# QData/LaMP

Measured on AMD Instinct MI355X. Metric: forward samples/sec, reuters d512 2+2L 4h, higher is better.
Workload: dtype f32

## Files before the change

include/lamp_hip.h:

```cpp
#ifndef LAMP_HIP_H
#define LAMP_HIP_H

#include <stddef.h>
#include <stdint.h>

#ifdef __cplusplus
extern "C" {
#endif
#if defined(__GNUC__)
#pragma GCC visibility push(default)
#endif

#define LAMP_HIP_ABI_VERSION 5

typedef void* lamp_stream_t;

enum lamp_status {
    LAMP_OK = 0,
    LAMP_E_DIMS = -1,
    LAMP_E_ALIGN = -2,
    LAMP_E_WORKSPACE = -3,
    LAMP_E_UNSUPPORTED = -4,
    LAMP_E_NULL = -5
};
// ... 314 lines not shown
    const float* slf_v;
} lamp_dec_gemm_pack;
typedef struct lamp_enc_gemm_pack {
    const float* w1;
    const float* w2;
} lamp_enc_gemm_pack;
typedef struct lamp_gemm_packs {
    const lamp_enc_gemm_pack* enc;
    const lamp_dec_gemm_pack* dec;
} lamp_gemm_packs;

int lamp_forward_packs(const lamp_model* m, const lamp_fwd_options* opts, const lamp_gemm_packs* packs, const int64_t* src_seq,
                       const int64_t* src_pos, int32_t B, int32_t T, float* logits, float* enc_output, const lamp_aux* aux,
                       void* workspace, size_t workspace_bytes, lamp_stream_t stream);

typedef struct lamp_onehot_frontend {
    const float* t1;
    const float* conv1_b;
    const float* conv2_w;
    const float* conv2_b;
    const float* conv2_pack;
    int32_t n_vocab;
    int32_t taps;
} lamp_onehot_frontend;

size_t lamp_onehot_forward_workspace_bytes(const lamp_model* m, const lamp_onehot_frontend* fe, int32_t micro_batch, int32_t T,
                                           int32_t want_attn);
int lamp_onehot_forward(const lamp_model* m, const lamp_onehot_frontend* fe, const int64_t* src_seq, const int64_t* src_pos,
                        int32_t B, int32_t T, float* logits, float* enc_output, const lamp_aux* aux, void* workspace,
                        size_t workspace_bytes, lamp_stream_t stream);
// ... 74 lines not shown
```

lamp_amd/Models.py:

```python
import ctypes as C

import collections

import torch
import torch.nn as nn

from . import _native as N
from .Decoders import GraphDecoder, MLPDecoder, RNNDecoder
from .Encoders import GraphEncoder, MLPEncoder, RNNEncoder
from .SubLayers import XavierLinear


def _chain_pack(fc, w1, w2, keep):
    ptrs = []
    for fmt in (0, 1):
        trio = [N.weight_pack(w, fmt) for w in (fc, w1, w2)]
        if any(t is None for t in trio):
            trio = [None] * 3
        keep.append(trio)
        ptrs += [N.ptr(t) for t in trio]
    return N.ChainPack(*ptrs)


class _MatmulPrecision:
# ... 166 lines not shown

    def _enc_chain_weights(self):
        out = []
        for l in self.encoder.layer_stack:
            if getattr(l.slf_attn, 'fc', None) is not None:
                out += [l.slf_attn.fc.weight, l.pos_ffn.w_1.weight, l.pos_ffn.w_2.weight]
        return out

    def _gemm_pack_weights(self):
        enc = [(l.pos_ffn.w_1.weight, l.pos_ffn.w_2.weight) for l in self.encoder.layer_stack]
        dec = []
        for l in self.decoder.layer_stack:
            slf = getattr(l, 'slf_attn', None)
            dec.append((l.enc_attn.w_qs.weight,) + (tuple(getattr(slf, n).weight for n in ('w_qs', 'w_ks', 'w_vs')) if slf is not None
                                                     else (None, None, None)))
        return enc, dec

    def _native_model(self):
        replica = getattr(self, '_is_replica', False)
        params = None if replica else self._param_list
        if params is None:
            params = self._weight_tensors()
            if not replica:
                self._param_list = params
        mask = self.decoder.label_mask_u8
        tiles = self.decoder.label_tiles
        bits = self.decoder.label_mask_bits
        bias = self.decoder.current_label_bias()
        if bias is not None:
            mask, tiles, bits = bias, None, None
        hoist = self.cache_layer0_query and not replica
        packs = self.use_chain_packs and not replica
        onehot = bool(getattr(self.encoder, 'onehot', False))
        live = self.enc_self_attn
        gpacks = bool(self.use_gemm_packs and not replica and not onehot and getattr(N.lib(), 'lamp_forward_packs', None))
        fold = self.fold_embedding and not replica and len(self.encoder.layer_stack) > 0 and not onehot and not live
        sparse = bool(self.use_sparse_label_attention and self.use_mask_bits and self.decoder.label_rows_sparse and bias is None)
        key = tuple(p.data_ptr() for p in params) + (N.ptr(mask), N.ptr(bits), N.ptr(tiles), self.use_label_tiles,
                                                      hoist, self.use_mask_bits, packs, fold, sparse, live, bias is not None, gpacks)
        if hoist:
            l0 = self.decoder.layer_stack[0].enc_attn
            key += (self.decoder.tgt_word_emb.weight._version, l0.w_qs.weight._version)
        if packs:
            key += tuple(w._version for w in self._chain_weights())
            if live:
                key += tuple(w._version for w in self._enc_chain_weights())
        if gpacks:
            key += tuple(w._version for group in self._gemm_pack_weights() for ws in group for w in ws if w is not None)
        if fold:
            key += tuple(w._version for w in self._fold_weights() if w is not None)
        if onehot:
            key += tuple((w.data_ptr(), w._version) for w in self._onehot_weights())
        cache = None if replica else self._native_cache
        if cache is not None and cache[0] == key:
# ... 36 lines not shown
                        continue
                    pack_arr[2 * i + j] = _chain_pack(att.fc.weight, ff.w_1.weight, ff.w_2.weight, pack_keep)
            m.chain_packs = pack_arr
            torch.cuda.current_stream().synchronize()
        enc_pack_arr = None
        if packs and live and len(enc.layer_stack) > 0:
            enc_pack_arr = (N.ChainPack * len(enc.layer_stack))()
            pack_keep = pack_keep if pack_keep is not None else []
            for i, l in enumerate(enc.layer_stack):
                if getattr(l.slf_attn, 'fc', None) is None:
                    continue
                enc_pack_arr[i] = _chain_pack(l.slf_attn.fc.weight, l.pos_ffn.w_1.weight, l.pos_ffn.w_2.weight, pack_keep)
            torch.cuda.current_stream().synchronize()
        gemm_keep = None
        if gpacks:
            enc_ws, dec_ws = self._gemm_pack_weights()
            tensors = []

            def pk(w):
                t = N.weight_pack(w, 0) if w is not None else None
                tensors.append(t)
                return N.ptr(t)
            enc_gp = (N.EncGemmPack * max(1, len(enc_ws)))(*[N.EncGemmPack(*[pk(w) for w in ws]) for ws in enc_ws])
            dec_gp = (N.DecGemmPack * max(1, len(dec_ws)))(*[N.DecGemmPack(*[pk(w) for w in ws]) for ws in dec_ws])
            gemm_keep = (N.GemmPacks(enc_gp, dec_gp), enc_gp, dec_gp, tensors)
            torch.cuda.current_stream().synchronize()
        fold_keep = None
        if fold:
            emb_w, pos_w, w1, b1 = self._fold_weights()
            w1 = w1.detach().reshape(w1.size(0), -1)
            e1 = N.linear(emb_w.detach(), w1, None if pos_w is not None else b1.detach())
            p1 = N.linear(pos_w.detach(), w1, b1.detach()) if pos_w is not None else None
            m.enc0_emb_w1, m.enc0_pos_w1 = e1.data_ptr(), N.ptr(p1)
            fold_keep = (e1, p1)
            torch.cuda.current_stream().synchronize()
        onehot_keep = None
        if onehot:
            e_w, w1, b1, w2, b2 = (w.detach() for w in self._onehot_weights())
            t1 = N.onehot_tap_table(e_w, w1)
            w2c, b1c, b2c = N.f32c(w2), N.f32c(b1), N.f32c(b2)
# ... 129 lines not shown
            def ws_bytes(mb):
                return lib.lamp_onehot_forward_workspace_bytes(C.byref(model), C.byref(fe), mb, T_in, int(want_attn))
        else:
            def ws_bytes(mb):
                return lib.lamp_forward_workspace_bytes(C.byref(model), mb, T, int(want_attn))
        per_sample = ws_bytes(1)
        fixed = 2 * per_sample - ws_bytes(2)
        whole = fixed + (per_sample - fixed) * B + 4096
        budget = max(per_sample + 4096, min(whole, self.workspace_limit_bytes))
        ws = N.workspace(budget, dev)
        if opts is not None and fe is not None:
            N.check(lib.lamp_onehot_forward_opts(C.byref(model), C.byref(fe), C.byref(opts), seq.data_ptr(), pos.data_ptr(), B,
                                                 T_in, logits.data_ptr(), enc_output.data_ptr(),
                                                 C.byref(aux) if aux is not None else None, ws.data_ptr(), ws.numel(),
                                                 N.stream()), 'lamp_onehot_forward_opts')
        elif gp is not None and fe is None:
            N.check(lib.lamp_forward_packs(C.byref(model), C.byref(opts) if opts is not None else None, C.byref(gp), seq.data_ptr(),
                                           pos.data_ptr(), B, T, logits.data_ptr(), enc_output.data_ptr(),
                                           C.byref(aux) if aux is not None else None, ws.data_ptr(), ws.numel(), N.stream()),
                    'lamp_forward_packs')
        elif opts is not None:
            N.check(lib.lamp_forward_opts(C.byref(model), C.byref(opts), seq.data_ptr(), pos.data_ptr(), B, T,
                                          logits.data_ptr(), enc_output.data_ptr(), C.byref(aux) if aux is not None else None,
                                          ws.data_ptr(), ws.numel(), N.stream()), 'lamp_forward_opts')
        elif fe is not None:
            N.check(lib.lamp_onehot_forward(C.byref(model), C.byref(fe), seq.data_ptr(), pos.data_ptr(), B, T_in,
                                            logits.data_ptr(), enc_output.data_ptr(), C.byref(aux) if aux is not None else None,
                                            ws.data_ptr(), ws.numel(), N.stream()), 'lamp_onehot_forward')
        else:
            N.check(lib.lamp_forward(C.byref(model), seq.data_ptr(), pos.data_ptr(), B, T, logits.data_ptr(),
# ... 14 lines not shown
        if was_training:
            self.eval()
        try:
            with torch.no_grad(), torch.cuda.device(src[0].device):
                logits = self.forward(src, adj, None, None)[0]
                idx, val = metrics.topk_labels(logits, k, values=True)
                return torch.sigmoid(val), idx.long()
        finally:
            if was_training:
                self.train(True)

    workspace_limit_bytes = 8 << 30
    cache_layer0_query = True
    use_chain_packs = True
    use_gemm_packs = True
    fold_embedding = True
    matmul_precision = _MatmulPrecision()
    use_packed_live_encoder = False
    use_label_tiles = True
    use_sparse_label_attention = True
    use_mask_bits = True
```

lamp_amd/_native.py:

```python
import ctypes as C
import os
import threading

import torch

_HERE = os.path.dirname(os.path.abspath(__file__))
LIB_PATH = os.environ.get('LAMP_HIP_LIBRARY') or os.path.join(_HERE, 'liblamp_hip.so')
TUNING_LIB_PATH = os.path.join(_HERE, 'liblamp_hip_tuning.so')

ABI_VERSION = 5
LAMP_MASK_NONE, LAMP_MASK_U8, LAMP_MASK_KEY_TOKENS_I64, LAMP_MASK_BITS_U32 = 0, 1, 2, 3
LAMP_MASK_BIAS_F32 = 4
LAMP_MASK_SPARSE_ROWS, LAMP_MASK_SELF_RAGGED = 1, 2
LAMP_FWD_PACKED_ENCODER, LAMP_FWD_DEC_SIGMOID = 1, 2
LAMP_FWD_MATMUL_BF16X3, LAMP_FWD_MATMUL_BF16X6 = 4, 8
LAMP_FWD_LABEL_BIAS = 16
LAMP_PREC_FP32, LAMP_PREC_BF16X3, LAMP_PREC_BF16X6 = 0, 1, 2
MATMUL_PRECISIONS = {'highest': (LAMP_PREC_FP32, 0), 'high': (LAMP_PREC_BF16X3, LAMP_FWD_MATMUL_BF16X3),
                     'bf16x6': (LAMP_PREC_BF16X6, LAMP_FWD_MATMUL_BF16X6)}
LAMP_ATTN_SOFTMAX, LAMP_ATTN_SIGMOID = 0, 1
ATTN_TYPES = {'softmax': LAMP_ATTN_SOFTMAX, 'sigmoid': LAMP_ATTN_SIGMOID}
K_EMBED, K_GEMM, K_ATTN, K_LAYERNORM, K_DIAG, K_COUNT = 0, 1, 2, 3, 4, 5
KERNEL_CLASS_NAMES = ('embed', 'gemm', 'attention', 'layernorm', 'diag_readout')

# ... 46 lines not shown
    _fields_ = [('n_src_vocab', C.c_int32), ('n_position', C.c_int32), ('n_labels', C.c_int32),
                ('d_model', C.c_int32), ('d_inner', C.c_int32), ('d_k', C.c_int32), ('d_v', C.c_int32),
                ('n_layers_enc', C.c_int32), ('n_layers_dec', C.c_int32), ('label_mask_flags', C.c_int32),
                ('src_word_emb', _vp), ('position_enc', _vp), ('tgt_word_emb', _vp), ('w_out', _vp),
                ('label_mask', _vp), ('label_mask_bits', _vp), ('label_tiles', _vp), ('enc_layers', C.POINTER(EncLayer)), ('dec_layers', C.POINTER(DecLayer)),
                ('dec0_query', _vp), ('chain_packs', C.POINTER(ChainPack)),
                ('enc0_emb_w1', _vp), ('enc0_pos_w1', _vp), ('label_mask_allowed', C.c_int64)]


class DecGemmPack(C.Structure):
    _fields_ = [('enc_q', _vp), ('slf_q', _vp), ('slf_k', _vp), ('slf_v', _vp)]


class EncGemmPack(C.Structure):
    _fields_ = [('w1', _vp), ('w2', _vp)]


class GemmPacks(C.Structure):
    _fields_ = [('enc', C.POINTER(EncGemmPack)), ('dec', C.POINTER(DecGemmPack))]


class GemmDesc(C.Structure):
    _fields_ = [('A', _vp), ('B', _vp), ('C', _vp), ('M', C.c_int32), ('N', C.c_int32), ('K', C.c_int32),
                ('batch0', C.c_int32), ('batch1', C.c_int32), ('accumulate', C.c_int32),
                ('a_row_stride', C.c_int64), ('a_col_stride', C.c_int64), ('a_batch0', C.c_int64), ('a_batch1', C.c_int64),
                ('b_row_stride', C.c_int64), ('b_col_stride', C.c_int64), ('b_batch0', C.c_int64), ('b_batch1', C.c_int64),
                ('ldc', C.c_int64), ('c_batch0', C.c_int64), ('c_batch1', C.c_int64),
                ('relu_mask', _vp), ('ld_mask', C.c_int64), ('alpha', C.c_float), ('reserved', C.c_int32)]


# ... 78 lines not shown
    'lamp_attn_bias_bwd': (C.c_int, [_vp, _i64, _i32, _i32, _f, _vp, _i64, _vp, _i64, _vp, _sz, _vp]),
    'lamp_label_bias_fold': (C.c_int, [_vp, _i64, _vp, _i32, _vp, _vp]),
    'lamp_dropout': (C.c_int, [_vp, _i64, _f, C.c_uint32, _vp, _vp]),
    'lamp_softmax_bwd': (C.c_int, [_vp, _vp, _i64, _i32, _f, _vp, _vp]),
    'lamp_diag_logits_bwd': (C.c_int, [_vp, _vp, _vp, _i32, _i32, _i32, _vp, _vp, _vp]),
    'lamp_embed_bwd': (C.c_int, [_vp, _i64, _vp, _i32, _i32, _i64, _vp, _vp]),
    'lamp_prior_graph_build': (C.c_int, [_vp, _vp, _i64, _i32, _vp, _vp, _vp]),
    'lamp_sigmoid_bce_fwd': (C.c_int, [_vp, _vp, _i64, _i32, _vp, _vp, _vp]),
    'lamp_forward_workspace_bytes': (_sz, [C.POINTER(Model), _i32, _i32, _i32]),
    'lamp_forward': (C.c_int, [C.POINTER(Model), _vp, _vp, _i32, _i32, _vp, _vp, C.POINTER(Aux), _vp, _sz, _vp]),
    'lamp_forward_opts_workspace_bytes': (_sz, [C.POINTER(Model), C.POINTER(FwdOptions), _i32, _i32, _i32]),
    'lamp_forward_opts': (C.c_int, [C.POINTER(Model), C.POINTER(FwdOptions), _vp, _vp, _i32, _i32, _vp, _vp, C.POINTER(Aux),
                                    _vp, _sz, _vp]),
    'lamp_forward_packs': (C.c_int, [C.POINTER(Model), C.POINTER(FwdOptions), C.POINTER(GemmPacks), _vp, _vp, _i32, _i32, _vp, _vp,
                                     C.POINTER(Aux), _vp, _sz, _vp]),
    'lamp_onehot_forward_opts_workspace_bytes': (_sz, [C.POINTER(Model), C.POINTER(OnehotFrontend), C.POINTER(FwdOptions),
                                                       _i32, _i32, _i32]),
    'lamp_onehot_forward_opts': (C.c_int, [C.POINTER(Model), C.POINTER(OnehotFrontend), C.POINTER(FwdOptions), _vp, _vp, _i32,
                                           _i32, _vp, _vp, C.POINTER(Aux), _vp, _sz, _vp]),
    'lamp_onehot_forward_workspace_bytes': (_sz, [C.POINTER(Model), C.POINTER(OnehotFrontend), _i32, _i32, _i32]),
    'lamp_onehot_forward': (C.c_int, [C.POINTER(Model), C.POINTER(OnehotFrontend), _vp, _vp, _i32, _i32, _vp, _vp,
                                      C.POINTER(Aux), _vp, _sz, _vp]),
    'lamp_conv_pack': (C.c_int, [_vp, _i32, _i32, _i32, _i32, _vp, _vp]),
    'lamp_onehot_front_fwd': (C.c_int, [_vp, _i32, _i32, C.POINTER(OnehotFrontend), _i32, _f, C.c_uint32, _vp, _vp]),
    'lamp_conv_window_fwd': (C.c_int, [_vp, _i32, _i32, _i32, _i32, _vp, _i32, _vp, _i32, _vp, _i32, _vp, _i64, _vp, _vp,
                                       _vp]),
    'lamp_conv_relu_bwd_pad': (C.c_int, [_vp, _vp, _i32, _i32, _i32, _vp, _vp]),
    'lamp_onehot_front_bwd_partials_bytes': (_sz, [_i32, _i32, _i32, _i32]),
    'lamp_onehot_front_bwd': (C.c_int, [_vp, _i32, _i32, C.POINTER(OnehotFrontend), _i32, _f, C.c_uint32, _vp, _vp, _vp,
                                        _sz, _vp]),
# ... 10 lines not shown
    'lamp_sdpa_act_fwd': (C.c_int, [_vp, _vp, _vp, _vp, _vp, _i32, _i32, _i32, _i32, _i32, _i32, _f, _i32,
                                    C.POINTER(Mask), C.POINTER(AttnLayout), _vp]),
    'lamp_mha_act_fwd': (C.c_int, [_vp, _vp, _i32, _i32, _i32, _i32, _i32, _i32, C.POINTER(MhaWeights), _i32,
                                   C.POINTER(Mask), _vp, _vp, _vp, _sz, _vp]),
    'lamp_mha_train_act_fwd': (C.c_int, [C.POINTER(MhaTrainDesc), C.POINTER(MhaWeights), _i32, _vp, _vp, _vp, C.POINTER(Mask)] +
                               [_vp] * 9 + [_vp]),
    'lamp_mha_act_bwd': (C.c_int, [C.POINTER(MhaTrainDesc), C.POINTER(MhaWeights), _i32] + [_vp] * 11 + [_vp] * 15 +
                         [_vp, _sz, _vp, _sz, C.POINTER(ReduceJob), _vp]),
    'lamp_sigmoid_attn_bwd': (C.c_int, [_vp, _vp, _i64, _i32, _f, _f, C.c_uint32, _vp, _vp]),
    'lamp_prof_enable': (C.c_int, [_i32]),
    'lamp_prof_reset': (C.c_int, []),
    'lamp_prof_read': (C.c_int, [_i32, C.POINTER(_i64), C.POINTER(C.c_double), C.POINTER(C.c_double),
                                 C.POINTER(C.c_double)]),
}

LATE_ENTRY_POINTS = ('lamp_linear_packed_fwd', 'lamp_forward_packs', 'lamp_attn_bias_bwd_workspace_bytes', 'lamp_attn_bias_bwd',
                     'lamp_label_bias_fold', 'lamp_topk_labels', 'lamp_rank_at_k_workspace_bytes', 'lamp_rank_at_k')

_lib = None
_lock = threading.Lock()


def load_library(path):
    if not os.path.exists(path):
        raise RuntimeError(
            'lamp_amd: %s is missing -- build it with `python -m lamp_amd.build` '
            '(hipcc, gfx950).  There is no CPU or PyTorch fallback.' % path)
    handle = C.CDLL(path)
    handle.lamp_version.restype = C.c_int
    version = handle.lamp_version()
    old_ok = version in (2, 3) and os.environ.get('LAMP_ALLOW_OLD_ABI') == '1'
# ... 878 lines not shown
```

lamp_amd/csrc/api.hip:

```cpp
#include <algorithm>
#include <mutex>
#include <vector>

#include "lamp_kernels.h"

namespace lamp {

namespace {
struct ProfRec {
    int cls;
    double flops, bytes;
    hipEvent_t e0, e1;
};
std::mutex g_prof_mu;
bool g_prof_on = false;
std::vector<ProfRec> g_prof;
std::vector<hipEvent_t> g_event_pool;
constexpr size_t PROF_MAX = 1 << 16;

hipEvent_t take_event() {
    if (!g_event_pool.empty()) {
        hipEvent_t e = g_event_pool.back();
        g_event_pool.pop_back();
        return e;
// ... 907 lines not shown
    int64_t b0;
    const int64_t *seq, *pos;
    int64_t ld_seq;
    float* x;
    bool packed;
    SeqPlan sp;
    lamp_mask pad_mask;
    lamp_mask label_mask;
    const float* xk = nullptr;
    int n_int = 0;
    const lamp_mask* enc_mask = nullptr;
    const lamp_chain_pack* enc_packs = nullptr;
    int dec_act = LAMP_ATTN_SOFTMAX;
    int prec = LAMP_PREC_FP32;
    const lamp_gemm_packs* gp = nullptr;
    void ffn_packs(FfnParams& f, int layer) const {
        if (gp && gp->enc) { f.w1_pack = gp->enc[layer].w1; f.w2_pack = gp->enc[layer].w2; }
    }
};

static int encode_packed(Pass& p) {
    const lamp_model* m = p.m;
    const FwdScratch& w = p.w;
    const int d = p.g.d, dff = p.g.dff, T = p.g.T;
    const bool folded = m->enc0_emb_w1 != nullptr;
    const bool gather_res =
        folded && gemm_gathered_residual_ok(d, dff, d, m->enc_layers[0].pos_ffn.b2, w.Xp, m->src_word_emb, m->position_enc);
    const EmbedFold fold{m->enc0_emb_w1, m->enc0_pos_w1, dff, folded ? w.H : nullptr, gather_res ? w.row_tok : nullptr,
                         gather_res ? w.row_pos : nullptr};
    const ResGather rg{w.row_tok, w.row_pos, m->src_word_emb, m->position_enc};
// ... 82 lines not shown
            continue;
        }
        if (map) {
            MhaCall a{p.x, p.x, p.nb, T, T, d, p.g.dk, p.g.dv, &l.slf_attn, p.enc_mask, nullptr, map, p.B, int(p.b0)};
            a.keys = &p.sp; a.prec = p.prec;
            LAMP_CK(mha_attend(a, w.mha, p.s));
        }
        f.hidden_ready = folded && i == 0;
        LAMP_CK(ffn_core(f, p.s));
    }
    p.xk = p.x;
    return 0;
}

static int project_kv_layers(const float* x, int64_t Me, int d, int dk, int dv, const lamp_dec_layer* layers, int n,
                             float* const* K, float* const* V, int prec, hipStream_t s, const int* m_dev, const float* A_dense) {
    const int h = layers[0].enc_attn.n_head;
    bool uniform = 2 * n <= GEMM_MAX_SEG && h * dk == h * dv;
    for (int i = 1; i < n && uniform; ++i) uniform = layers[i].enc_attn.n_head == h;
    if (uniform) {
        const float* W[GEMM_MAX_SEG];
        float* C[GEMM_MAX_SEG];
        for (int i = 0; i < n; ++i) {
            if (!layers[i].enc_attn.w_ks || !layers[i].enc_attn.w_vs) return LAMP_E_NULL;
            W[2 * i] = layers[i].enc_attn.w_ks;
            W[2 * i + 1] = layers[i].enc_attn.w_vs;
            C[2 * i] = K[i];
            C[2 * i + 1] = V[i];
        }
        return linear(x, Me, d, d, W, 2 * n, h * dk, d, nullptr, nullptr, 0, 0, C, h * dk, prec, s, m_dev, A_dense);
    }
    for (int i = 0; i < n; ++i)
        LAMP_CK(project_qkv(layers[i].enc_attn, d, dk, dv, nullptr, 0, nullptr, x, x, Me, K[i], V[i], prec, s, m_dev, A_dense));
    return 0;
}

static int int_pred(Pass& p) {
    const lamp_aux* a = p.aux;
    const int n = p.n_int++;
    if (!a || !a->int_preds || n >= a->n_int_preds || !a->int_preds[n]) return 0;
    return launch_diag(p.w.Y, p.m->w_out, p.nb, p.g.L, p.g.d, a->int_preds[n] + p.b0 * p.g.L, p.s);
}

static int decoder_layer(Pass& p, int i) {
    const lamp_model* m = p.m;
    const FwdDims& g = p.g;
    const FwdScratch& w = p.w;
    const lamp_dec_layer& l = m->dec_layers[i];
// ... 5 lines not shown
    bool ffn_ran = false;
    FfnParams f1{Y, Md, d, dff, &l.pos_ffn1, Y, w.H}, f2{Y, Md, d, dff, &l.pos_ffn2, Y, w.H};
    f2.n_labels = L;
    f1.prec = f2.prec = p.prec;
    const bool fused_readout = last && !g.live;
    if (fused_readout) { f2.w_out = m->w_out; f2.logits = p.logits + p.b0 * L; }

    MhaScratch sc = w.mha;
    if (g.n_ahead) { sc.K = w.K_ahead[i]; sc.V = w.V_ahead[i]; }
    MhaCall enc{i == 0 ? m->tgt_word_emb : Y, p.xk, p.nb, L, g.T, d, g.dk, g.dv, &l.enc_attn, &p.pad_mask, Y,
                p.aux && p.aux->dec_enc_attn ? p.aux->dec_enc_attn[i] : nullptr, p.B, int(p.b0)};
    enc.xq_shared = i == 0; enc.q_ready = i == 0 ? m->dec0_query : nullptr; enc.kv_ready = g.n_ahead > 0;
    enc.keys = &p.sp; enc.keys_packed = p.packed; enc.xkv_dense = p.x;
    enc.act = p.dec_act; enc.prec = p.prec;
    const lamp_dec_gemm_pack* dp = p.gp && p.gp->dec ? p.gp->dec + i : nullptr;
    const float* enc_pk[3] = {dp ? dp->enc_q : nullptr, nullptr, nullptr};
    const float* slf_pk[3] = {dp ? dp->slf_q : nullptr, dp ? dp->slf_k : nullptr, dp ? dp->slf_v : nullptr};
    enc.w_packs = enc_pk;
    LAMP_CK(mha_attend(enc, sc, p.s));
    LAMP_CK(mha_tail(enc, sc, &f1, pk, &ffn_ran, p.s));
    if (!ffn_ran) LAMP_CK(ffn_core(f1, p.s));

    ffn_ran = false;
    if (l.slf_attn.present) {
        LAMP_CK(int_pred(p));
        MhaCall slf{Y, Y, p.nb, L, L, d, g.dk, g.dv, &l.slf_attn, &p.label_mask, Y,
                    p.aux && p.aux->dec_self_attn ? p.aux->dec_self_attn[i] : nullptr, p.B, int(p.b0)};
        slf.act = p.dec_act; slf.prec = p.prec; slf.w_packs = slf_pk;
        LAMP_CK(mha_attend(slf, w.mha, p.s));
        LAMP_CK(mha_tail(slf, w.mha, &f2, pk ? pk + 1 : nullptr, &ffn_ran, p.s));
    }
// ... 41 lines not shown
        if ((o->flags & LAMP_FWD_DEC_SIGMOID) || m->label_mask_bits || m->label_tiles || m->label_mask_flags ||
            m->label_mask_allowed)
            return LAMP_E_UNSUPPORTED;
        if (m->label_mask && !aligned16(m->label_mask)) return LAMP_E_ALIGN;
    }
    if ((m->d_model & 3) || (m->d_inner & 3) || (m->d_k & 3) || (m->d_v & 3)) return LAMP_E_UNSUPPORTED;
    if (fe && ((fe->conv2_pack && !aligned16(fe->conv2_pack)) || (!fe->conv2_pack && !aligned16(fe->conv2_w)) ||
               !aligned16(fe->t1) || !aligned16(fe->conv1_b) || !aligned16(workspace)))
        return LAMP_E_ALIGN;
    return 0;
}

static int forward(const lamp_model* m, const lamp_onehot_frontend* fe, const FwdDims& g, const int64_t* src_seq,
                   const int64_t* src_pos, int32_t B, int32_t T_in, float* logits, float* enc_output, const lamp_aux* aux,
                   void* workspace, size_t workspace_bytes, hipStream_t s, const lamp_fwd_options* o = nullptr,
                   const lamp_gemm_packs* gp = nullptr) {
    const Carver size = fwd_size(g);
    if (workspace_bytes < size.bound(1)) return LAMP_E_WORKSPACE;
    const int64_t mb = std::min<int64_t>(B, (workspace_bytes - size.fixed) / size.per);
    Carver c{static_cast<char*>(workspace), size_t(mb)};
    FwdScratch w{};
    fwd_layout(g, c, w);
    if (fe) {
        if (g.w2_repack) LAMP_CK(launch_conv_pack(fe->conv2_w, g.d, g.d, 16, 0, w.w2, s));
        else w.w2 = const_cast<float*>(fe->conv2_pack);
    }

    bool packed_live = g.live && o && (o->flags & LAMP_FWD_PACKED_ENCODER) && !o->enc_mask && g.dk == g.dv &&
                       attn_ragged_applies(g.T, g.dk, g.dv);
    for (int i = 0; i < m->n_layers_enc && packed_live; ++i) packed_live = m->enc_layers[i].slf_attn.n_head > 1;
    const bool packed = !(aux && aux->enc_self_attn) && !wide_heads(g.dk, g.dv) && m->n_layers_enc > 0 && !fe &&
// ... 14 lines not shown
        Pass p{m, fe, g, w, aux, logits, s, B, nb, b0, seq, src_pos ? src_pos + b0 * T_in : nullptr, T_in,
               enc_output + b0 * int64_t(g.T) * g.d, packed, plan_from(w.plan_ints, nb, g.T),
               lamp_mask{LAMP_MASK_KEY_TOKENS_I64, 0, seq, T_in, 0, nullptr, 0}, label_mask};
        p.sp.granules = packed ? w.granules : nullptr;
        lamp_mask enc_mask = p.pad_mask;
        if (o && o->enc_mask) {
            enc_mask = *o->enc_mask;
            enc_mask.ptr = static_cast<const uint8_t*>(enc_mask.ptr) + b0 * enc_mask.stride_b;
        }
        if (g.live) enc_mask.flags |= LAMP_MASK_SELF_RAGGED;
        p.enc_mask = &enc_mask;
        p.enc_packs = o ? o->enc_chain_packs : nullptr;
        p.dec_act = (o && (o->flags & LAMP_FWD_DEC_SIGMOID)) ? LAMP_ATTN_SIGMOID : LAMP_ATTN_SOFTMAX;
        p.prec = fwd_matmul_prec(o);
        p.gp = gp;
        LAMP_CK(!packed ? encode_padded(p) : g.live ? encode_packed_live(p) : encode_packed(p));
        if (g.n_ahead)
            LAMP_CK(project_kv_layers(p.xk, int64_t(nb) * g.T, g.d, g.dk, g.dv, m->dec_layers, g.n_ahead, w.K_ahead,
                                      w.V_ahead, p.prec, s, packed ? p.sp.rows : nullptr, packed ? p.x : nullptr));
        for (int i = 0; i < m->n_layers_dec; ++i) LAMP_CK(decoder_layer(p, i));
    }
    return 0;
}

size_t lamp_forward_workspace_bytes(const lamp_model* m, int32_t micro_batch, int32_t T, int32_t want_attn) {
    FwdDims g;
    if (micro_batch <= 0 || fwd_dims(m, nullptr, T, want_attn != 0, &g) != 0) return 0;
    return fwd_size(g).bound(micro_batch);
}

static int forward_tokens(const lamp_model* m, const lamp_fwd_options* o, const int64_t* src_seq, const int64_t* src_pos,
                          int32_t B, int32_t T, float* logits, float* enc_output, const lamp_aux* aux, void* workspace,
                          size_t workspace_bytes, lamp_stream_t stream, const lamp_gemm_packs* gp = nullptr) {
    FwdDims g;
    LAMP_CK(check_forward(m, nullptr, src_seq, src_pos, B, T, logits, enc_output, aux, workspace, &g, o));
    if (workspace_bytes < fwd_size(g).bound(1)) return LAMP_E_WORKSPACE;
    const bool kv_ahead =
        2 * m->n_layers_dec <= GEMM_MAX_SEG && m->n_layers_dec > 1 && workspace_bytes >= fwd_size(g).bound(size_t(B));
    if (!kv_ahead) g.n_ahead = 0;
    return forward(m, nullptr, g, src_seq, src_pos, B, T, logits, enc_output, aux, workspace, workspace_bytes,
                   hipStream_t(stream), o, gp);
}

int lamp_forward(const lamp_model* m, const int64_t* src_seq, const int64_t* src_pos, int32_t B, int32_t T,
                 float* logits, float* enc_output, const lamp_aux* aux, void* workspace, size_t workspace_bytes,
                 lamp_stream_t stream) {
    return forward_tokens(m, nullptr, src_seq, src_pos, B, T, logits, enc_output, aux, workspace, workspace_bytes, stream);
}

size_t lamp_forward_opts_workspace_bytes(const lamp_model* m, const lamp_fwd_options* opts, int32_t micro_batch, int32_t T,
                                         int32_t want_attn) {
    FwdDims g;
    if (micro_batch <= 0 || fwd_dims(m, nullptr, T, want_attn != 0, &g, opts && opts->enc_self_attn) != 0) return 0;
    return fwd_size(g).bound(micro_batch);
}

int lamp_forward_opts(const lamp_model* m, const lamp_fwd_options* opts, const int64_t* src_seq, const int64_t* src_pos,
                      int32_t B, int32_t T, float* logits, float* enc_output, const lamp_aux* aux, void* workspace,
                      size_t workspace_bytes, lamp_stream_t stream) {
    return forward_tokens(m, opts, src_seq, src_pos, B, T, logits, enc_output, aux, workspace, workspace_bytes, stream);
}

int lamp_forward_packs(const lamp_model* m, const lamp_fwd_options* opts, const lamp_gemm_packs* packs, const int64_t* src_seq,
                       const int64_t* src_pos, int32_t B, int32_t T, float* logits, float* enc_output, const lamp_aux* aux,
                       void* workspace, size_t workspace_bytes, lamp_stream_t stream) {
    return forward_tokens(m, opts, src_seq, src_pos, B, T, logits, enc_output, aux, workspace, workspace_bytes, stream, packs);
}

size_t lamp_onehot_forward_workspace_bytes(const lamp_model* m, const lamp_onehot_frontend* fe, int32_t micro_batch, int32_t T,
                                           int32_t want_attn) {
    FwdDims g;
    if (micro_batch <= 0 || onehot_check(m, fe, T) != 0 || fwd_dims(m, fe, T, want_attn != 0, &g) != 0) return 0;
    return fwd_size(g).bound(micro_batch);
}

int lamp_onehot_forward(const lamp_model* m, const lamp_onehot_frontend* fe, const int64_t* src_seq, const int64_t* src_pos,
                        int32_t B, int32_t T, float* logits, float* enc_output, const lamp_aux* aux, void* workspace,
                        size_t workspace_bytes, lamp_stream_t stream) {
    return lamp_onehot_forward_opts(m, fe, nullptr, src_seq, src_pos, B, T, logits, enc_output, aux, workspace, workspace_bytes,
                                    stream);
}
// ... 102 lines not shown
```

lamp_amd/csrc/gemm.hip:

```cpp
#include <type_traits>

#include "lamp_kernels.h"

namespace lamp {

struct FastDiv {
    unsigned mul, shift;
};
static inline FastDiv make_fastdiv(unsigned d) {
    if (d <= 1) return FastDiv{0u, 0u};
    unsigned l = 0;
    while ((1ull << l) < d) ++l;
    return FastDiv{unsigned(((1ull << (31 + l)) + d - 1) / d), l - 1};
}
__device__ __forceinline__ int fdiv(int n, FastDiv f) { return f.mul ? int(__umulhi(unsigned(n), f.mul) >> f.shift) : n; }
__device__ __forceinline__ int div_1_to_8(int n, int d) {
    if ((d & (d - 1)) == 0) return n >> (31 - __builtin_clz(unsigned(d)));
    const unsigned mul = d == 5 ? 0xCCCCCCCDu : (d == 7 ? 0x92492493u : 0xAAAAAAABu);
    return int(__umulhi(unsigned(n), mul) >> (d == 3 ? 1 : 2));
}

constexpr int gemm_min_waves(int bm, int bn, int bk, int mf, bool wpack = false) {
    return (wpack || (mf == 16 && bm == 64 && bn == 64 && bk == 16)) ? 5 : 1;
}

template <int BM, int BN, int BK, int WAVES_M, int WAVES_N, int MF = 32, bool WPACK = false>
struct GemmTile {
    static constexpr int NT = WAVES_M * WAVES_N * 64;
    static constexpr int WTM = BM / WAVES_M;
    static constexpr int WTN = BN / WAVES_N;
    static constexpr int MI = WTM / MF;
    static constexpr int NI = WTN / MF;
#ifndef LAMP_LDS_PAD16
#define LAMP_LDS_PAD16 8
#endif
    static constexpr int LDS_STRIDE = BK + (MF == 16 ? LAMP_LDS_PAD16 : 4);
    static constexpr int A_LD = BM * BK / 4 / NT;
    static constexpr int B_LD = BN * BK / 4 / NT;
    static constexpr size_t LDS_BYTES = size_t(2) * (BM + (WPACK ? 0 : BN)) * LDS_STRIDE * sizeof(float);
    static constexpr size_t LDS_LAUNCH_BYTES = WPACK ? size_t(2) * (BM + BN) * LDS_STRIDE * sizeof(float) : LDS_BYTES;
    static constexpr int MIN_WAVES = gemm_min_waves(BM, BN, BK, MF, WPACK);
    static_assert(MF == 32 || MF == 16, "MFMA block edge");
    static_assert(WTM % MF == 0 && WTN % MF == 0, "wave tile must be a multiple of the MFMA block");
    static_assert(BK % (MF == 32 ? 8 : 16) == 0, "BK must cover whole fragment reads");
    static_assert((BM * BK / 4) % NT == 0 && (BN * BK / 4) % NT == 0, "staging must divide evenly");
    static_assert(BK % 8 == 0, "BK must be a multiple of 8");
};


__device__ __forceinline__ const float* uniform_ptr(const float* q) {
    const uint64_t b = reinterpret_cast<uint64_t>(q);
    const unsigned lo = __builtin_amdgcn_readfirstlane(unsigned(b)), hi = __builtin_amdgcn_readfirstlane(unsigned(b >> 32));
    return reinterpret_cast<const float*>((uint64_t(hi) << 32) | lo);
}
template <int BM, int BN, int BK, int WAVES_M, int WAVES_N, bool KTAIL, int MF, bool RPRE, bool VEC, bool RGATHER, bool WPACK>
// ... 429 lines not shown

template <int BM, int BN, int BK, int WAVES_M, int WAVES_N, int MF = 32>
static int launch_cfg(const GemmParams& p, hipStream_t s) {
    if (p.rg_tok) {
        if (!p.vec_epilogue || (p.K % BK)) return LAMP_E_UNSUPPORTED;
        return launch_cfg2<BM, BN, BK, WAVES_M, WAVES_N, false, MF, true, true>(p, s);
    }
    if (p.vec_epilogue) {
        if (p.K % BK) return launch_cfg2<BM, BN, BK, WAVES_M, WAVES_N, true, MF, true>(p, s);
        return launch_cfg2<BM, BN, BK, WAVES_M, WAVES_N, false, MF, true>(p, s);
    }
    if (p.K % BK) return launch_cfg2<BM, BN, BK, WAVES_M, WAVES_N, true, MF, false>(p, s);
    return launch_cfg2<BM, BN, BK, WAVES_M, WAVES_N, false, MF, false>(p, s);
}

static int launch_packed(const GemmParams& p, hipStream_t s) {
    if (p.rg_tok) return launch_cfg2<32, 64, 32, 1, 4, false, 16, true, true, true>(p, s);
    return launch_cfg2<32, 64, 32, 1, 4, false, 16, true, false, true>(p, s);
}

static bool gemm_packed_ok(const GemmParams& p) {
    if (!p.vec_epilogue || (p.N & 15) || (p.K & 31) || (int64_t(p.N) + 64) * p.K * 4 >= 0x7fffffffLL) return false;
    for (int i = 0; i < p.nseg; ++i)
        if (!p.Wp[i] || !aligned16(p.Wp[i])) return false;
    return true;
}

#ifdef LAMP_TUNING
static int g_force_tile = 0;
static unsigned long long* g_gemm_trace = nullptr;
static long long g_trace_slab = 0;
static int g_trace_slabs = 0, g_trace_count = 0;
extern "C" __attribute__((visibility("default"))) void lamp_debug_force_gemm_tile(int cfg) { g_force_tile = cfg; }
extern "C" __attribute__((visibility("default"))) void lamp_debug_set_gemm_trace(unsigned long long* buf, long long slab_words, int n_slabs) {
// ... 33 lines not shown
#ifdef LAMP_TUNING
    if (g_gemm_trace && g_trace_slabs > 0) {
        const long long wg_max = ((p.M + 31) / 32) * ((p.N + 63) / 64) * p.nseg;
        if (wg_max * 8 <= g_trace_slab) p.trace = g_gemm_trace + (g_trace_count % g_trace_slabs) * g_trace_slab;
        ++g_trace_count;
    }
    switch (g_force_tile) {
        case 1: return launch_cfg<128, 128, 32, 2, 2>(p, s);
        case 2: return launch_cfg<64, 64, 32, 2, 2>(p, s);
        case 3: return launch_cfg<128, 64, 32, 2, 2>(p, s);
        case 4: return launch_cfg<64, 128, 32, 2, 2>(p, s);
        case 5: return launch_cfg<128, 128, 16, 2, 2>(p, s);
        case 6: return launch_cfg<64, 64, 16, 2, 2>(p, s);
        case 7: return launch_cfg<128, 64, 16, 2, 2>(p, s);
        case 8: return launch_cfg<256, 128, 16, 4, 2>(p, s);
        case 9: return gemm_packed_ok(p) ? launch_packed(p, s) : launch_cfg<32, 64, 32, 1, 4, 16>(p, s);
        case 10: return launch_cfg<64, 32, 32, 4, 1, 16>(p, s);
        case 11: return launch_cfg<64, 64, 16, 2, 2, 16>(p, s);
        case 12: return launch_cfg<64, 64, 32, 2, 2, 16>(p, s);
        case 13: return launch_cfg<32, 128, 32, 1, 4, 16>(p, s);
        case 14: return launch_cfg<128, 128, 32, 2, 2, 16>(p, s);
        case 15: return launch_cfg<128, 128, 16, 2, 2, 16>(p, s);
        case 16: return launch_cfg<128, 64, 32, 2, 2, 16>(p, s);
        case 17: return launch_cfg<64, 128, 32, 2, 2, 16>(p, s);
        case 18: return launch_cfg<128, 64, 16, 2, 2, 16>(p, s);
        default: break;
    }
#endif
    auto tiles = [&](int bm, int bn) { return ((p.M + bm - 1) / bm) * ((p.N + bn - 1) / bn) * p.nseg; };
    const int64_t t64 = tiles(64, 64);
    if (tiles(128, 64) >= 2048 && p.K >= 512) return launch_cfg<128, 64, 16, 2, 2, 16>(p, s);
    if (t64 >= 2048) return launch_cfg<64, 64, 32, 2, 2, 16>(p, s);
#ifndef LAMP_PACKED_FFN_TILE
#define LAMP_PACKED_FFN_TILE 1
#endif
    const bool packed = gemm_packed_ok(p);
    if (t64 >= 1200 && !(LAMP_PACKED_FFN_TILE && packed)) return launch_cfg<64, 64, 16, 2, 2, 16>(p, s);
    if (packed) return launch_packed(p, s);
    return launch_cfg<32, 64, 32, 1, 4, 16>(p, s);
}

}
```

Measured before the change: 45980.

## Use pre-packed weights for encoder-attention K/V projections and add tall packed GEMM tile

Adds packed weight layouts for the decoder's encoder-attention K and V projection weights and routes them through a new forward entry point, so those GEMMs can use the packed-weight kernel path. It also adds a 64-row packed GEMM tile for large non-token-gathered problems when wave quantization looks favorable, and adjusts LDS and occupancy settings for the wider packed variants. The aim is cheaper weight loads for the K/V projections and better tile choice on large GEMMs. The cost is extra packed weight memory, another API path, and heuristic risk in the tile selection.

```diff
diff --git a/include/lamp_hip.h b/include/lamp_hip.h
--- a/include/lamp_hip.h
+++ b/include/lamp_hip.h
@@ -352,6 +352,15 @@
                        const int64_t* src_pos, int32_t B, int32_t T, float* logits, float* enc_output, const lamp_aux* aux,
                        void* workspace, size_t workspace_bytes, lamp_stream_t stream);
 
+typedef struct lamp_kv_gemm_pack {
+    const float* enc_k;
+    const float* enc_v;
+} lamp_kv_gemm_pack;
+
+int lamp_forward_packs_kv(const lamp_model* m, const lamp_fwd_options* opts, const lamp_gemm_packs* packs, const lamp_kv_gemm_pack* kv_packs,
+                          const int64_t* src_seq, const int64_t* src_pos, int32_t B, int32_t T, float* logits, float* enc_output,
+                          const lamp_aux* aux, void* workspace, size_t workspace_bytes, lamp_stream_t stream);
+
 typedef struct lamp_onehot_frontend {
     const float* t1;
     const float* conv1_b;
diff --git a/lamp_amd/Models.py b/lamp_amd/Models.py
--- a/lamp_amd/Models.py
+++ b/lamp_amd/Models.py
@@ -204,7 +204,8 @@
             slf = getattr(l, 'slf_attn', None)
             dec.append((l.enc_attn.w_qs.weight,) + (tuple(getattr(slf, n).weight for n in ('w_qs', 'w_ks', 'w_vs')) if slf is not None
                                                      else (None, None, None)))
-        return enc, dec
+        kv = [(l.enc_attn.w_ks.weight, l.enc_attn.w_vs.weight) for l in self.decoder.layer_stack]
+        return enc, dec, kv
 
     def _native_model(self):
         replica = getattr(self, '_is_replica', False)
@@ -224,10 +225,11 @@
         onehot = bool(getattr(self.encoder, 'onehot', False))
         live = self.enc_self_attn
         gpacks = bool(self.use_gemm_packs and not replica and not onehot and getattr(N.lib(), 'lamp_forward_packs', None))
+        kvpacks = bool(gpacks and self.use_kv_gemm_packs and getattr(N.lib(), 'lamp_forward_packs_kv', None))
         fold = self.fold_embedding and not replica and len(self.encoder.layer_stack) > 0 and not onehot and not live
         sparse = bool(self.use_sparse_label_attention and self.use_mask_bits and self.decoder.label_rows_sparse and bias is None)
         key = tuple(p.data_ptr() for p in params) + (N.ptr(mask), N.ptr(bits), N.ptr(tiles), self.use_label_tiles,
-                                                      hoist, self.use_mask_bits, packs, fold, sparse, live, bias is not None, gpacks)
+                                                      hoist, self.use_mask_bits, packs, fold, sparse, live, bias is not None, gpacks, kvpacks)
         if hoist:
             l0 = self.decoder.layer_stack[0].enc_attn
             key += (self.decoder.tgt_word_emb.weight._version, l0.w_qs.weight._version)
@@ -294,7 +296,7 @@
             torch.cuda.current_stream().synchronize()
         gemm_keep = None
         if gpacks:
-            enc_ws, dec_ws = self._gemm_pack_weights()
+            enc_ws, dec_ws, kv_ws = self._gemm_pack_weights()
             tensors = []
 
             def pk(w):
@@ -303,7 +305,10 @@
                 return N.ptr(t)
             enc_gp = (N.EncGemmPack * max(1, len(enc_ws)))(*[N.EncGemmPack(*[pk(w) for w in ws]) for ws in enc_ws])
             dec_gp = (N.DecGemmPack * max(1, len(dec_ws)))(*[N.DecGemmPack(*[pk(w) for w in ws]) for ws in dec_ws])
-            gemm_keep = (N.GemmPacks(enc_gp, dec_gp), enc_gp, dec_gp, tensors)
+            kv_gp = None
+            if kvpacks:
+                kv_gp = (N.KvGemmPack * max(1, len(kv_ws)))(*[N.KvGemmPack(*[pk(w) for w in ws]) for ws in kv_ws])
+            gemm_keep = (N.GemmPacks(enc_gp, dec_gp), enc_gp, dec_gp, tensors, kv_gp)
             torch.cuda.current_stream().synchronize()
         fold_keep = None
         if fold:
@@ -463,6 +468,11 @@
                                                  T_in, logits.data_ptr(), enc_output.data_ptr(),
                                                  C.byref(aux) if aux is not None else None, ws.data_ptr(), ws.numel(),
                                                  N.stream()), 'lamp_onehot_forward_opts')
+        elif gp is not None and fe is None and built[9][4] is not None:
+            N.check(lib.lamp_forward_packs_kv(C.byref(model), C.byref(opts) if opts is not None else None, C.byref(gp), built[9][4],
+                                              seq.data_ptr(), pos.data_ptr(), B, T, logits.data_ptr(), enc_output.data_ptr(),
+                                              C.byref(aux) if aux is not None else None, ws.data_ptr(), ws.numel(), N.stream()),
+                    'lamp_forward_packs_kv')
         elif gp is not None and fe is None:
             N.check(lib.lamp_forward_packs(C.byref(model), C.byref(opts) if opts is not None else None, C.byref(gp), seq.data_ptr(),
                                            pos.data_ptr(), B, T, logits.data_ptr(), enc_output.data_ptr(),
@@ -507,6 +517,7 @@
     cache_layer0_query = True
     use_chain_packs = True
     use_gemm_packs = True
+    use_kv_gemm_packs = True
     fold_embedding = True
     matmul_precision = _MatmulPrecision()
     use_packed_live_encoder = False
diff --git a/lamp_amd/_native.py b/lamp_amd/_native.py
--- a/lamp_amd/_native.py
+++ b/lamp_amd/_native.py
@@ -84,6 +84,10 @@
 
 class EncGemmPack(C.Structure):
     _fields_ = [('w1', _vp), ('w2', _vp)]
+
+
+class KvGemmPack(C.Structure):
+    _fields_ = [('enc_k', _vp), ('enc_v', _vp)]
 
 
 class GemmPacks(C.Structure):
@@ -192,6 +196,8 @@
                                     _vp, _sz, _vp]),
     'lamp_forward_packs': (C.c_int, [C.POINTER(Model), C.POINTER(FwdOptions), C.POINTER(GemmPacks), _vp, _vp, _i32, _i32, _vp, _vp,
                                      C.POINTER(Aux), _vp, _sz, _vp]),
+    'lamp_forward_packs_kv': (C.c_int, [C.POINTER(Model), C.POINTER(FwdOptions), C.POINTER(GemmPacks), C.POINTER(KvGemmPack), _vp, _vp, _i32,
+                                        _i32, _vp, _vp, C.POINTER(Aux), _vp, _sz, _vp]),
     'lamp_onehot_forward_opts_workspace_bytes': (_sz, [C.POINTER(Model), C.POINTER(OnehotFrontend), C.POINTER(FwdOptions),
                                                        _i32, _i32, _i32]),
     'lamp_onehot_forward_opts': (C.c_int, [C.POINTER(Model), C.POINTER(OnehotFrontend), C.POINTER(FwdOptions), _vp, _vp, _i32,
@@ -232,7 +238,7 @@
                                  C.POINTER(C.c_double)]),
 }
 
-LATE_ENTRY_POINTS = ('lamp_linear_packed_fwd', 'lamp_forward_packs', 'lamp_attn_bias_bwd_workspace_bytes', 'lamp_attn_bias_bwd',
+LATE_ENTRY_POINTS = ('lamp_linear_packed_fwd', 'lamp_forward_packs', 'lamp_forward_packs_kv', 'lamp_attn_bias_bwd_workspace_bytes', 'lamp_attn_bias_bwd',
                      'lamp_label_bias_fold', 'lamp_topk_labels', 'lamp_rank_at_k_workspace_bytes', 'lamp_rank_at_k')
 
 _lib = None
diff --git a/lamp_amd/csrc/api.hip b/lamp_amd/csrc/api.hip
--- a/lamp_amd/csrc/api.hip
+++ b/lamp_amd/csrc/api.hip
@@ -945,6 +945,7 @@
     int dec_act = LAMP_ATTN_SOFTMAX;
     int prec = LAMP_PREC_FP32;
     const lamp_gemm_packs* gp = nullptr;
+    const lamp_kv_gemm_pack* kvp = nullptr;
     void ffn_packs(FfnParams& f, int layer) const {
         if (gp && gp->enc) { f.w1_pack = gp->enc[layer].w1; f.w2_pack = gp->enc[layer].w2; }
     }
@@ -1057,24 +1058,30 @@
 }
 
 static int project_kv_layers(const float* x, int64_t Me, int d, int dk, int dv, const lamp_dec_layer* layers, int n,
-                             float* const* K, float* const* V, int prec, hipStream_t s, const int* m_dev, const float* A_dense) {
+                             float* const* K, float* const* V, int prec, hipStream_t s, const int* m_dev, const float* A_dense,
+                             const lamp_kv_gemm_pack* packs = nullptr) {
     const int h = layers[0].enc_attn.n_head;
     bool uniform = 2 * n <= GEMM_MAX_SEG && h * dk == h * dv;
     for (int i = 1; i < n && uniform; ++i) uniform = layers[i].enc_attn.n_head == h;
     if (uniform) {
         const float* W[GEMM_MAX_SEG];
         float* C[GEMM_MAX_SEG];
+        const float* Wp[GEMM_MAX_SEG];
         for (int i = 0; i < n; ++i) {
             if (!layers[i].enc_attn.w_ks || !layers[i].enc_attn.w_vs) return LAMP_E_NULL;
             W[2 * i] = layers[i].enc_attn.w_ks;
             W[2 * i + 1] = layers[i].enc_attn.w_vs;
             C[2 * i] = K[i];
             C[2 * i + 1] = V[i];
+            Wp[2 * i] = packs ? packs[i].enc_k : nullptr;
+            Wp[2 * i + 1] = packs ? packs[i].enc_v : nullptr;
         }
-        return linear(x, Me, d, d, W, 2 * n, h * dk, d, nullptr, nullptr, 0, 0, C, h * dk, prec, s, m_dev, A_dense);
-    }
-    for (int i = 0; i < n; ++i)
-        LAMP_CK(project_qkv(layers[i].enc_attn, d, dk, dv, nullptr, 0, nullptr, x, x, Me, K[i], V[i], prec, s, m_dev, A_dense));
+        return linear(x, Me, d, d, W, 2 * n, h * dk, d, nullptr, nullptr, 0, 0, C, h * dk, prec, s, m_dev, A_dense, nullptr, Wp);
+    }
+    for (int i = 0; i < n; ++i) {
+        const float* Wp[3] = {nullptr, packs ? packs[i].enc_k : nullptr, packs ? packs[i].enc_v : nullptr};
+        LAMP_CK(project_qkv(layers[i].enc_attn, d, dk, dv, nullptr, 0, nullptr, x, x, Me, K[i], V[i], prec, s, m_dev, A_dense, Wp));
+    }
     return 0;
 }
 
@@ -1110,7 +1117,8 @@
     enc.keys = &p.sp; enc.keys_packed = p.packed; enc.xkv_dense = p.x;
     enc.act = p.dec_act; enc.prec = p.prec;
     const lamp_dec_gemm_pack* dp = p.gp && p.gp->dec ? p.gp->dec + i : nullptr;
-    const float* enc_pk[3] = {dp ? dp->enc_q : nullptr, nullptr, nullptr};
+    const lamp_kv_gemm_pack* kp = p.kvp ? p.kvp + i : nullptr;
+    const float* enc_pk[3] = {dp ? dp->enc_q : nullptr, kp ? kp->enc_k : nullptr, kp ? kp->enc_v : nullptr};
     const float* slf_pk[3] = {dp ? dp->slf_q : nullptr, dp ? dp->slf_k : nullptr, dp ? dp->slf_v : nullptr};
     enc.w_packs = enc_pk;
     LAMP_CK(mha_attend(enc, sc, p.s));
@@ -1182,7 +1190,7 @@
 static int forward(const lamp_model* m, const lamp_onehot_frontend* fe, const FwdDims& g, const int64_t* src_seq,
                    const int64_t* src_pos, int32_t B, int32_t T_in, float* logits, float* enc_output, const lamp_aux* aux,
                    void* workspace, size_t workspace_bytes, hipStream_t s, const lamp_fwd_options* o = nullptr,
-                   const lamp_gemm_packs* gp = nullptr) {
+                   const lamp_gemm_packs* gp = nullptr, const lamp_kv_gemm_pack* kvp = nullptr) {
     const Carver size = fwd_size(g);
     if (workspace_bytes < size.bound(1)) return LAMP_E_WORKSPACE;
     const int64_t mb = std::min<int64_t>(B, (workspace_bytes - size.fixed) / size.per);
@@ -1227,10 +1235,12 @@
         p.dec_act = (o && (o->flags & LAMP_FWD_DEC_SIGMOID)) ? LAMP_ATTN_SIGMOID : LAMP_ATTN_SOFTMAX;
         p.prec = fwd_matmul_prec(o);
         p.gp = gp;
+        p.kvp = kvp;
         LAMP_CK(!packed ? encode_padded(p) : g.live ? encode_packed_live(p) : encode_packed(p));
         if (g.n_ahead)
             LAMP_CK(project_kv_layers(p.xk, int64_t(nb) * g.T, g.d, g.dk, g.dv, m->dec_layers, g.n_ahead, w.K_ahead,
-                                      w.V_ahead, p.prec, s, packed ? p.sp.rows : nullptr, packed ? p.x : nullptr));
+                                      w.V_ahead, p.prec, s, packed ? p.sp.rows : nullptr, packed ? p.x : nullptr,
+                                      kvp));
         for (int i = 0; i < m->n_layers_dec; ++i) LAMP_CK(decoder_layer(p, i));
     }
     return 0;
@@ -1244,7 +1254,8 @@
 
 static int forward_tokens(const lamp_model* m, const lamp_fwd_options* o, const int64_t* src_seq, const int64_t* src_pos,
                           int32_t B, int32_t T, float* logits, float* enc_output, const lamp_aux* aux, void* workspace,
-                          size_t workspace_bytes, lamp_stream_t stream, const lamp_gemm_packs* gp = nullptr) {
+                          size_t workspace_bytes, lamp_stream_t stream, const lamp_gemm_packs* gp = nullptr,
+                          const lamp_kv_gemm_pack* kvp = nullptr) {
     FwdDims g;
     LAMP_CK(check_forward(m, nullptr, src_seq, src_pos, B, T, logits, enc_output, aux, workspace, &g, o));
     if (workspace_bytes < fwd_size(g).bound(1)) return LAMP_E_WORKSPACE;
@@ -1252,7 +1263,7 @@
         2 * m->n_layers_dec <= GEMM_MAX_SEG && m->n_layers_dec > 1 && workspace_bytes >= fwd_size(g).bound(size_t(B));
     if (!kv_ahead) g.n_ahead = 0;
     return forward(m, nullptr, g, src_seq, src_pos, B, T, logits, enc_output, aux, workspace, workspace_bytes,
-                   hipStream_t(stream), o, gp);
+                   hipStream_t(stream), o, gp, kvp);
 }
 
 int lamp_forward(const lamp_model* m, const int64_t* src_seq, const int64_t* src_pos, int32_t B, int32_t T,
@@ -1278,6 +1289,12 @@
                        const int64_t* src_pos, int32_t B, int32_t T, float* logits, float* enc_output, const lamp_aux* aux,
                        void* workspace, size_t workspace_bytes, lamp_stream_t stream) {
     return forward_tokens(m, opts, src_seq, src_pos, B, T, logits, enc_output, aux, workspace, workspace_bytes, stream, packs);
+}
+
+int lamp_forward_packs_kv(const lamp_model* m, const lamp_fwd_options* opts, const lamp_gemm_packs* packs, const lamp_kv_gemm_pack* kv_packs,
+                          const int64_t* src_seq, const int64_t* src_pos, int32_t B, int32_t T, float* logits, float* enc_output,
+                          const lamp_aux* aux, void* workspace, size_t workspace_bytes, lamp_stream_t stream) {
+    return forward_tokens(m, opts, src_seq, src_pos, B, T, logits, enc_output, aux, workspace, workspace_bytes, stream, packs, kv_packs);
 }
 
 size_t lamp_onehot_forward_workspace_bytes(const lamp_model* m, const lamp_onehot_frontend* fe, int32_t micro_batch, int32_t T,
diff --git a/lamp_amd/csrc/gemm.hip b/lamp_amd/csrc/gemm.hip
--- a/lamp_amd/csrc/gemm.hip
+++ b/lamp_amd/csrc/gemm.hip
@@ -20,8 +20,11 @@
     return int(__umulhi(unsigned(n), mul) >> (d == 3 ? 1 : 2));
 }
 
+#ifndef LAMP_PACKED_128_WAVES
+#define LAMP_PACKED_128_WAVES 4
+#endif
 constexpr int gemm_min_waves(int bm, int bn, int bk, int mf, bool wpack = false) {
-    return (wpack || (mf == 16 && bm == 64 && bn == 64 && bk == 16)) ? 5 : 1;
+    return (wpack && bm == 128) ? LAMP_PACKED_128_WAVES : (wpack || (mf == 16 && bm == 64 && bn == 64 && bk == 16)) ? 5 : 1;
 }
 
 template <int BM, int BN, int BK, int WAVES_M, int WAVES_N, int MF = 32, bool WPACK = false>
@@ -38,7 +41,7 @@
     static constexpr int A_LD = BM * BK / 4 / NT;
     static constexpr int B_LD = BN * BK / 4 / NT;
     static constexpr size_t LDS_BYTES = size_t(2) * (BM + (WPACK ? 0 : BN)) * LDS_STRIDE * sizeof(float);
-    static constexpr size_t LDS_LAUNCH_BYTES = WPACK ? size_t(2) * (BM + BN) * LDS_STRIDE * sizeof(float) : LDS_BYTES;
+    static constexpr size_t LDS_LAUNCH_BYTES = (WPACK && BM == 32) ? size_t(2) * (BM + BN) * LDS_STRIDE * sizeof(float) : LDS_BYTES;
     static constexpr int MIN_WAVES = gemm_min_waves(BM, BN, BK, MF, WPACK);
     static_assert(MF == 32 || MF == 16, "MFMA block edge");
     static_assert(WTM % MF == 0 && WTN % MF == 0, "wave tile must be a multiple of the MFMA block");
@@ -498,10 +501,15 @@
     return launch_cfg2<BM, BN, BK, WAVES_M, WAVES_N, false, MF, false>(p, s);
 }
 
+template <int BM = 32>
 static int launch_packed(const GemmParams& p, hipStream_t s) {
-    if (p.rg_tok) return launch_cfg2<32, 64, 32, 1, 4, false, 16, true, true, true>(p, s);
-    return launch_cfg2<32, 64, 32, 1, 4, false, 16, true, false, true>(p, s);
-}
+    if (p.rg_tok) return launch_cfg2<BM, 64, 32, 1, 4, false, 16, true, true, true>(p, s);
+    return launch_cfg2<BM, 64, 32, 1, 4, false, 16, true, false, true>(p, s);
+}
+
+#ifdef LAMP_TUNING
+static int launch_packed_128(const GemmParams& p, hipStream_t s) { return launch_cfg2<128, 64, 32, 1, 4, false, 16, true, false, true>(p, s); }
+#endif
 
 static bool gemm_packed_ok(const GemmParams& p) {
     if (!p.vec_epilogue || (p.N & 15) || (p.K & 31) || (int64_t(p.N) + 64) * p.K * 4 >= 0x7fffffffLL) return false;
@@ -565,7 +573,7 @@
         case 6: return launch_cfg<64, 64, 16, 2, 2>(p, s);
         case 7: return launch_cfg<128, 64, 16, 2, 2>(p, s);
         case 8: return launch_cfg<256, 128, 16, 4, 2>(p, s);
-        case 9: return gemm_packed_ok(p) ? launch_packed(p, s) : launch_cfg<32, 64, 32, 1, 4, 16>(p, s);
+        case 9: return gemm_packed_ok(p) ? launch_packed<32>(p, s) : launch_cfg<32, 64, 32, 1, 4, 16>(p, s);
         case 10: return launch_cfg<64, 32, 32, 4, 1, 16>(p, s);
         case 11: return launch_cfg<64, 64, 16, 2, 2, 16>(p, s);
         case 12: return launch_cfg<64, 64, 32, 2, 2, 16>(p, s);
@@ -575,19 +583,31 @@
         case 16: return launch_cfg<128, 64, 32, 2, 2, 16>(p, s);
         case 17: return launch_cfg<64, 128, 32, 2, 2, 16>(p, s);
         case 18: return launch_cfg<128, 64, 16, 2, 2, 16>(p, s);
+        case 19: if (gemm_packed_ok(p)) return launch_packed<64>(p, s); break;
+        case 20: if (gemm_packed_ok(p)) return p.rg_tok ? launch_packed<64>(p, s) : launch_packed_128(p, s); break;
         default: break;
     }
 #endif
     auto tiles = [&](int bm, int bn) { return ((p.M + bm - 1) / bm) * ((p.N + bn - 1) / bn) * p.nseg; };
     const int64_t t64 = tiles(64, 64);
+    const bool packed = gemm_packed_ok(p);
+#ifndef LAMP_PACKED_TALL_TILE
+#define LAMP_PACKED_TALL_TILE 1
+#endif
+#ifndef LAMP_PACKED_TALL_MIN_TILES
+#define LAMP_PACKED_TALL_MIN_TILES 2048
+#endif
+    if (LAMP_PACKED_TALL_TILE && packed && !p.rg_tok && t64 >= LAMP_PACKED_TALL_MIN_TILES && tiles(128, 64) < 4096) {
+        const int64_t rounds = (t64 + 1279) / 1280;
+        if (5 * t64 >= 4 * rounds * 1280) return launch_cfg2<64, 64, 32, 1, 4, false, 16, true, false, true>(p, s);
+    }
     if (tiles(128, 64) >= 2048 && p.K >= 512) return launch_cfg<128, 64, 16, 2, 2, 16>(p, s);
     if (t64 >= 2048) return launch_cfg<64, 64, 32, 2, 2, 16>(p, s);
 #ifndef LAMP_PACKED_FFN_TILE
 #define LAMP_PACKED_FFN_TILE 1
 #endif
-    const bool packed = gemm_packed_ok(p);
     if (t64 >= 1200 && !(LAMP_PACKED_FFN_TILE && packed)) return launch_cfg<64, 64, 16, 2, 2, 16>(p, s);
-    if (packed) return launch_packed(p, s);
+    if (packed) return launch_packed<32>(p, s);
     return launch_cfg<32, 64, 32, 1, 4, 16>(p, s);
 }
 
```

Result: faster. 46470, median of 6 (+1.1%).
